# kaiidams/voice100

Measured on AMD Instinct MI355X. Metric: audio frames/sec (fwd+bwd) asr_en_base, B=32x1024-frame mel, higher is better.
Workload: dtype bf16

## Files before the change

### include/voice100_hip.h

```cpp
#ifndef VOICE100_HIP_H
#define VOICE100_HIP_H

#ifdef __cplusplus
extern "C" {
#endif


int v100_dw_num_groups(int B, int C);
int v100_dwconv(const float* x, const float* x2, const float* w, const float* in_a, const float* in_b,
                const float* in_c, int in_mode, float* y, const float* aux, const float* out_a,
                const float* out_b, int out_mode, float* stats, int G, int B, int C, int Tin, int Tout,
                int K, int stride, int pad, int flip, int upsample, int force_generic, void* stream);

int v100_dwconv_wgrad(const float* g, const float* g2, const float* ga, const float* gb, const float* gc,
                      int g_mode, const float* x, const float* xa, const float* xb, int x_mode,
                      float* partial, float* dw, int G, int B, int C, int Tin, int Tout, int K, int stride,
                      int pad, int force_generic, void* stream);

int v100_dwconv_bwd(const float* g, const float* g2, const float* w, const float* ga, const float* gb,
                    const float* gc, const float* xpre, const float* xa, const float* xb, float* dxin,
                    float* stats, float* wpartial, float* dw, int G, int B, int C, int Tin, int Tout, int K,
                    int stride, int pad, int force_split, void* stream);

int v100_pw_num_parts(int B, int T);
int v100_pw_gemm(const float* A, const void* A_bf16, const float* X, const float* X2, const float* xa,
                 const float* xb, const float* xc, int x_mode, float* Y, const float* bias, const float* ea,
                 const float* eb, const float* R, int epi_mode, float* stats, int B, int M, int K, int T,
                 int use_bf16, void* stream);
int v100_pw_gemm_dropmask_supported(int B, int M, int K, int T, int use_bf16);
int v100_pw_gemm_dropmask(const float* A, const void* A_bf16, const float* X, float* Y, const void* keep, float p, int B, int M, int K,
                          int T, int use_bf16, void* stream);

int v100_pw_wgrad_splits(int B, int M, int K);
int v100_pw_wgrad(const float* G, const float* G2, const float* ga, const float* gb, const float* gc, int g_mode,
                  const float* X, const float* xa, const float* xb, int x_mode, float* partial, float* dW,
                  int S, int B, int M, int K, int T, int use_bf16, void* stream);

int v100_weight_prep(const float* w, int rows, int cols, void* w_bf16, float* wt, void* wt_bf16, void* stream);
int v100_weight_prep_f16(const float* w, int rows, int cols, void* w16, void* stream);

int v100_bn_finalize_train(const float* stats, int parts, long long count, const float* gamma, const float* beta,
                           float* running_mean, float* running_var, long long* num_batches_tracked, float momentum,
                           float eps, float* scale, float* shift, float* save_mean, float* save_rstd, int C, void* stream);
int v100_bn_eval_coeffs(const float* gamma, const float* beta, const float* running_mean, const float* running_var,
                        float eps, float* scale, float* shift, int C, void* stream);
int v100_bn_bwd_finalize(const float* partial, int parts, long long count, const float* gamma, const float* mean,
                         const float* rstd, float* p, float* q, float* r, float* dgamma, float* dbeta, int C, void* stream);
int v100_bn_frozen_coeffs(const float* gamma, const float* beta, const float* running_mean, const float* running_var,
                          float eps, float* scale, float* shift, float* mean, float* rstd, int C, void* stream);
int v100_bn_bwd_finalize_frozen(const float* partial, int parts, long long count, const float* gamma, const float* mean,
                                const float* rstd, float* p, float* q, float* r, float* dgamma, float* dbeta, int C, void* stream);

int v100_chan_reduce2(const float* u, const float* v, float* partial, int G, int B, int C, int T, void* stream);
int v100_slab_sum0(const float* partial, int parts, float* out, int C, void* stream);
int v100_chan_affine2(const float* u, const float* v, const float* A, const float* Bc, const float* Cc, float* out,
                      int B, int C, int T, void* stream);
int v100_mul_scale(const float* u, const float* m, float s, float* out, long long n, void* stream);
int v100_dropout_fwd(const float* x, long long seed, float p, float* y, void* mask, long long n, void* stream);
int v100_dropout_bwd(const float* dy, const void* mask, float p, float* dx, long long n, void* stream);
int v100_transpose_last2(const float* in, float* out, int B, int R, int Cc, void* stream);
int v100_embedding_bct(const long long* idx, const float* table, float* out, int B, int V, int C, int T, void* stream);
int v100_embedding_bwd(const long long* idx, const float* g, float* dtable, int B, int V, int C, int T, void* stream);


int v100_augment_fused(const float* x, const int* len, const float* uniform, float* y, int B, int Tin, int Tout,
                       int F, int stretch_rate, float pitch_rate, float amp, int n_tmask, const int* tm_s,
                       const int* tm_e, const float* tm_a, int fm_on, int fm_s, int fm_e, float fm_a, int noise_on,
                       float noise_low, float noise_high, float noise_std, int mix, float log_offset, void* stream);
int v100_augment_fused_len(const float* x, const int* len_raw, int* len_out, int* half_out, const float* uniform, float* y,
                           int B, int Tin, int Tout, int F, int stretch_rate, float pitch_rate, float amp, int n_tmask,
                           const int* tm_s, const int* tm_e, const float* tm_a, int fm_on, int fm_s, int fm_e, float fm_a,
                           int noise_on, float noise_low, float noise_high, float noise_std, int mix, float log_offset,
                           void* stream);
int v100_augment_fused_len_t(const float* x, const int* len_raw, int* len_out, int* half_out, const float* uniform, float* y,
                             float* yt, int B, int Tin, int Tout, int F, int stretch_rate, float pitch_rate, float amp, int n_tmask,
                             const int* tm_s, const int* tm_e, const float* tm_a, int fm_on, int fm_s, int fm_e, float fm_a,
                             int noise_on, float noise_low, float noise_high, float noise_std, int mix, float log_offset,
                             void* stream);

int v100_shift_copy(const float* in, float* out, const float* bias, int B, int C, int Tin, int Tout, int in_ctot,
                    int in_coff, int out_ctot, int out_coff, int in_mul, int in_add, int out_mul, int out_add, int n,
                    int accumulate, void* stream);
int v100_stft_frames(const float* x, float* frames, int B, int N, int T, int hop, int win, int n_fft, void* stream);
int v100_power_spectrum(const float* spec, float* pw, int B, int F, int T, void* stream);
int v100_log_transpose(const float* in, float* out, int B, int C, int T, float offset, void* stream);
int v100_log_mel_fused(const float* x, float* out, const float* window, const float* tw256, const float* tw512, const int* mel_start,
                       const int* mel_count, const float* mel_w, int B, int N, int T, int hop, int n_fft, int n_mels, float log_offset,
                       void* stream);
int v100_log_mel_fused_len(const float* x, const int* lengths, float* out, int* out_len, const float* window, const float* tw256,
                           const float* tw512, const int* mel_start, const int* mel_count, const float* mel_w, int B, int N, int T,
                           int hop, int n_fft, int n_mels, float log_offset, float fill, void* stream);
int v100_world_unnormalize(const float* x, float* f0, float* logspc, float* codeap, const float* f0_mean, const float* f0_std,
                           const float* ls_mean, const float* ls_std, const float* ca_mean, const float* ca_std,
                           int B, int T, int S, int Cap, void* stream);
int v100_world_loss_parts(int B, int Tp);
int v100_world_loss(const float* pred, const float* f0, const float* hasf0, const float* logspc, const float* codeap,
                    const int* length, const float* f0_mean, const float* f0_std, const float* ls_mean, const float* ls_std,
                    const float* ca_mean, const float* ca_std, const float* w, float* partial, float* loss, float* unit,
                    int B, int Tp, int Tt, int S, int Cap, int l1, void* stream);
int v100_world_loss_bwd(const float* unit, const float* gout, float* dpred, int B, int Tp, int S, int Cap, void* stream);
int v100_exp_clip(const float* x, float* y, float offset, long long n, void* stream);

int v100_bct_to_cm(const float* in, float* out, int B, int C, int T, void* stream);
int v100_cm_to_btc(const float* in, float* out, int B, int C, int T, void* stream);

int v100_world_randn_host(float* host_out, long long n);
int v100_world_decode_aperiodicity(const float* coded, float* ap, long long rows, int nb, int fs, int fft_size, void* stream);
long long v100_world_synth_workspace_bytes(int B, int T, int fs, double frame_period_ms, int fft_size, int max_pulses);
int v100_world_synthesize(const float* f0, const float* sp, const float* ap, const float* coded_ap, int nb, const int* frames, const float* randn_table,
                          long long table_len, const float* tw256, const float* tw512, const float* dc_remover, float* y,
                          int* n_pulses, void* workspace, int B, int T, int fs, double frame_period_ms, int fft_size,
                          int max_pulses, void* stream);

int v100_im2col(const float* x, float* cols, int B, int Cin, int Tin, int Tout, int k, int stride, int pad, void* stream);
int v100_col2im(const float* dcols, float* dx, int B, int Cin, int Tin, int Tout, int k, int stride, int pad, void* stream);
int v100_pad_copy(const float* src, float* dst, int B, int C, int Tsrc, int src_step, int src_off, int n, int Tx, int lpad, void* stream);
int v100_pw_taps_supported(int B, int M, int cx, int ntap, int T, int Tx, int use_bf16);
int v100_pw_gemm_taps(const float* A, const void* A_bf16, const float* Xp, float* Y, const float* bias, const float* R,
                      int B, int M, int cx, int T, int Tx, int ntap, const int* shifts, int use_bf16, void* stream);
int v100_pw_wgrad_taps(const float* G, int Tg, int g_off, const float* Xp, float* partial, float* dW, int S, int B, int M,
                       int cx, int T, int Tx, int ntap, const int* shifts, int use_bf16, void* stream);
int v100_ln_num_parts(int B, int T);
int v100_slab_sum2(const float* partial, int parts, float* out0, float* out1, int C, void* stream);
int v100_ln_gelu_fwd(const float* y, const float* gamma, const float* beta, float eps, float* out, float* mean,
                     float* rstd, int B, int C, int T, void* stream);
int v100_ln_gelu_bwd(const float* dout, const float* y, const float* gamma, const float* beta, const float* mean,
                     const float* rstd, float* dy, float* partial, int B, int C, int T, void* stream);

long long v100_launch_count(void);
int v100_copy_probe(const void* src, void* dst, long long nbytes, void* stream);
int v100_timing_enable(int tag_mask);
int v100_timing_read(int tag, double* ms, long long* count, double* bytes);
int v100_rows_copy_probe(const void* src, void* dst, int B, int C, int row_bytes, void* stream);

int v100_pw_gemm_io(const void* A_bf16, const void* X, const void* X2, const float* xa, const float* xb, const float* xc,
                    int x_mode, void* Y, const float* ea, const float* eb, const void* R, int epi_mode, float* stats,
                    int B, int M, int K, int T, int io16, void* stream);
int v100_pw_wgrad_io(const void* G, const void* G2, const float* ga, const float* gb, const float* gc, int g_mode,
                     const void* X, const float* xa, const float* xb, int x_mode, float* partial, float* dW, int S, int B,
                     int M, int K, int T, int io16, void* stream);
int v100_pw_wgrad_group_supported(int B, int M, int K, int T, int S, int g_mode, int x_mode, int io16);
int v100_pw_wgrad_group_tiles(int M, int K, int x_mode);
int v100_pw_wgrad_group(int n, const void* const* ptrs, const int* dims, void* stream);
int v100_pw_wgrad_group_small_supported(int B, int M, int K, int T, int S, int g_mode, int x_mode, int io16);
int v100_pw_wgrad_group_small_tiles(int M, int K, int x_mode);
int v100_pw_wgrad_group_small(int n, const void* const* ptrs, const int* dims, void* stream);
int v100_dw_mfma_supported(int K, int stride);
int v100_row_pitch16(int T, int B);
int v100_dwconv_fwd_train_io(const void* a1, const float* w, const float* in_a, const float* in_b, void* a2, float* stats,
                             int G, int B, int C, int T, int K, int io16, void* stream);
int v100_dwconv_bwd_io(const void* g, const void* g2, const float* w, const float* ga, const float* gb, const float* gc,
                       const void* xpre, const float* xa, const float* xb, void* dxin, float* stats, float* wpartial,
                       float* dw, int G, int B, int C, int T, int K, int io16, void* stream);
int v100_dwconv_bwd_da1_io(const void* g, const void* g2, const float* w, const float* ga, const float* gb, const float* gc,
                           const void* xpre, const float* xa, const float* xb, void* da1_out, float* stats, float* dw,
                           const float* bn1_gamma, const float* bn1_mean, const float* bn1_rstd, float* pqr, float* dgamma,
                           float* dbeta, int B, int C, int T, int K, void* stream);
int v100_dwconv_fwd_eval_io(const void* h1, const float* w, const float* out_a, const float* out_b, void* h2, int B, int C, int T,
                            int K, int flags, void* stream);
int v100_chan_reduce2_io(const void* u, const void* v, float* partial, int G, int B, int C, int T, int io16, void* stream);
int v100_chan_affine2_shadow(const void* u, const float* v, const float* A, const float* Cc, float* out, void* shadow,
                             int B, int C, int T, int u_bf16, void* stream);
int v100_chan_affine2_io(const void* u, const void* v, const float* A, const float* Bc, const float* Cc, void* out,
                         int B, int C, int T, int io16, void* stream);
int v100_ir_act16_supported(const int* shape);

int v100_adam_chunk_elems(void);
int v100_adam_step(const void* chunks, int nchunks, const void* params, const void* grads, const void* exp_avg,
                   const void* exp_avg_sq, double lr, double beta1, double beta2, double eps, double weight_decay, int step,
                   void* stream);

int v100_grad_norm_partials(const void* chunks, int nchunks, const void* grads, void* partials, int norm_type, void* stream);
int v100_adam_step_clip(const void* chunks, int nchunks, const void* params, const void* grads, const void* exp_avg,
                        const void* exp_avg_sq, double lr, double beta1, double beta2, double eps, double weight_decay, int step,
                        int clip_mode, double clip, const void* partials, int npartials, int norm_type, void* total_norm, void* stream);
int v100_grad_clip(const void* chunks, int nchunks, const void* grads, int clip_mode, double clip, const void* partials, int npartials,
                   int norm_type, void* total_norm, void* stream);

int v100_ctc_workspace_floats(int B, int T, int Lmax);
int v100_ctc_loss_mean(const float* logits, const long long* targets, const int* in_len, const int* tgt_len, float* workspace,
                       float* nll, float* loss, float* grad, int B, int T, int V, int Lmax, int blank, void* stream);
int v100_ctc_loss(const float* logits, const long long* targets, const int* in_len, const int* tgt_len, float* workspace,
                  float* nll, float* grad, int B, int T, int V, int Lmax, int blank, void* stream);
int v100_ctc_loss_mean_t(const float* logits, const long long* targets, const int* in_len, const int* tgt_len, float* workspace,
                         float* nll, float* loss, float* grad, int grad_bvt, int B, int T, int V, int Lmax, int blank, void* stream);

enum {
    V100_IR_PREPPED = 1,
    V100_IR_SHADOW_SLOTS = 2,
    V100_IR_FROZEN = 8
};
long long v100_ir_prep_bytes(const int* shape);
long long v100_ir_fwd_workspace_bytes(const int* shape);
long long v100_ir_eval_cache_bytes(const int* shape);
int v100_ir_eval_prep(const int* shape, const void* const* ptrs, void* stream);
int v100_ir_fwd_eval(const int* shape, const void* const* ptrs, void* stream);
int v100_ir_stack_fwd_eval(int n, const int* shapes, const void* const* ptrs, void* stream);
int v100_ir_prep_batched(const int* shapes, const void* const* w1s, const void* const* w3s, void* const* preps, int n, void* stream);
int v100_ir_fwd_train(const int* shape, const void* const* ptrs, void* stream);
long long v100_ir_bwd_workspace_bytes(const int* shape);
int v100_ir_bwd(const int* shape, const void* const* ptrs, void* stream);

long long v100_ir_stack_plan(const int* desc, long long* plan);
int v100_ir_stack_fwd_train(const int* desc, const void* const* params, const void* x, const void* x16, void* blob, void* stream);
int v100_ir_stack_bwd(const int* desc, const void* const* params, const void* x, const void* x16, const void* blob, const void* dy,
                      void* dx, void* grads, void* ws, void* stream);
int v100_ir_stack_wgrad_plan(const int* desc, int have_x16, int min_problem_tiles, int min_flush_tiles, long long* out);
int v100_ir_stack_wgrad_group_thresholds(int min_problem_tiles, int min_flush_tiles);
int v100_ir_stack_wgrad_plan2(const int* desc, int have_x16, int min_problem_tiles, int min_flush_tiles, int min_flush_small, long long* out);
int v100_ir_stack_wgrad_group2_threshold(int min_flush_small);

int v100_ctc_greedy_decode(const float* logits, const int* lens, long long* out, int* out_len, int B, int T, int V, int blank, void* stream);
int v100_ctc_best_path(const float* logp, const long long* labels, const int* in_len, const int* lab_len, void* back_ws, int* path,
                       float* score, int B, int T, int V, int Lmax, int max_move, void* stream);
long long v100_ctc_align_workspace_bytes(int B, int T, int Lmax);
int v100_ctc_align_block(void);
int v100_ctc_align(const float* logp, const long long* labels, const int* in_len, const int* lab_len, void* moves_ws, int* path,
                   long long* best_labels, int* align, float* score, int B, int T, int V, int Lmax, int max_move, void* stream);
long long v100_ctc_align_long_workspace_bytes(int B, int T, int Lmax, int band);
int v100_ctc_align_long_block(void);
int v100_ctc_align_long(const float* logp, const long long* labels, const int* in_len, const int* lab_len, const float* free_logp, void* ws,
                        double* score, int* ok, int* path, int* align, int B, int T, int V, int Lmax, int band, int blank, void* stream);
long long v100_ctc_cut_points_workspace_bytes(int B, int T);
int v100_ctc_cut_points_span(void);
int v100_ctc_cut_points_pass(void);
int v100_ctc_cut_points(const float* logits, const int* lengths, void* ws, int* n_seg, int B, int T, int V, int blank, int max_frames,
                        int min_gap, float margin, int pad, int min_frames, void* stream);
int v100_ctc_cut_points_table(const void* ws, int* start, int* end, int* forced, int B, int T, int S, int pad, void* stream);
long long v100_edit_distance_workspace_bytes(int B, int Th, int Tr);
int v100_edit_distance(const long long* hyp, const int* hyp_len, const long long* ref, const int* ref_len, void* ws, int* dist,
                       int* hyp_n, int* ref_n, long long* totals, int B, int Th, int Tr, int levels, long long sep, void* stream);
long long v100_ctc_beam_workspace_bytes(int B, int T, int V, int W);
int v100_ctc_beam_search(const float* logits, const int* lens, void* ws, long long* ids, int* ids_len, float* scores, int B, int T, int V,
                         int W, int nbest, int blank, void* stream);
int v100_ctc_beam_search_lm(const float* logits, const int* lens, void* ws, long long* ids, int* ids_len, float* scores,
                            const float* lm_logp, const int* lm_next, const float* lm_final, int S, int start_state, float alpha,
                            float beta, int use_eos, float* ctc_scores, float* lm_scores, int B, int T, int V, int W, int nbest,
                            int blank, void* stream);
long long v100_ctc_beam_stream_workspace_bytes(int B, int max_frames, int V, int W);
long long v100_ctc_beam_stream_state_bytes(int B, int W);
int v100_ctc_beam_stream_push(const float* logits, const int* lens, void* ws, void* state, int B, int T, int max_frames, int V, int W,
                              int blank, void* stream);
int v100_ctc_beam_stream_push_lm(const float* logits, const int* lens, void* ws, void* state, const float* lm_logp, const int* lm_next,
                                 const float* lm_final, int S, int start_state, float alpha, float beta, int B, int T, int max_frames,
                                 int V, int W, int blank, void* stream);
int v100_ctc_beam_stream_read(const void* ws, const void* state, long long* ids, int* ids_len, float* scores, int B, int max_frames,
                              int V, int W, int nbest, int width, void* stream);
int v100_ctc_beam_stream_read_lm(const void* ws, const void* state, long long* ids, int* ids_len, float* scores, const float* lm_final,
                                 int S, int start_state, float alpha, float beta, int final, float* ctc_scores, float* lm_scores, int B,
                                 int max_frames, int V, int W, int nbest, int width, void* stream);
long long v100_ctc_segment_workspace_bytes(int B, int T, int Lmax);
int v100_ctc_segment_block(void);
int v100_ctc_segment(const float* logits, const int* in_len, const long long* labels, const int* lab_len, void* ws, float* log_prob,
                     int* start, int* end, float* duration, float* log_conf, int* word_first, int* word_count, int* word_start,
                     int* word_end, float* word_log_conf, int* n_words, int B, int T, int V, int Lmax, int blank, long long sep,
                     void* stream);
long long v100_dtw_workspace_bytes(int B, int Tx, int Ty, int D, int want_path);
int v100_dtw_score(const float* x, const int* x_len, const float* y, const int* y_len, const float* f0x, const float* f0y, void* ws,
                   double* cost, int* path_len, int* voiced, int* vuv_errors, double* f0_sq_cents, double* f0_sq_hz, int* path,
                   double* totals, int B, int Tx, int Ty, int D, int skip, float f0_floor, int mode, void* stream);
int v100_align_expand(const long long* text, const double* align, const int* text_len, long long* out, int* out_len, int B, int Lmax,
                      int Tmax, int head, int tail, void* stream);


int v100_world_randn_host_f64(double* host_out, long long n);
long long v100_world_randn_bound(int kind, int T, int fs, int fft_size);
int v100_world_frames(int fs, int length, double frame_period_ms);
int v100_world_dio_bands(int fs, double f0_floor, double f0_ceil, double channels_in_octave, int* half_lengths, int max_bands);
long long v100_world_dio_workspace_bytes(int B, int max_len, int fs, double f0_floor, double f0_ceil, double channels_in_octave,
                                         double frame_period_ms);
int v100_world_dio(const float* x, const int* lengths, int B, int max_len, int pitch, int fs, double f0_floor, double f0_ceil,
                   double channels_in_octave, double frame_period_ms, double allowed_range, const double* lowcut,
                   const double* nuttall, double* f0, void* workspace, void* stream);
int v100_world_cheaptrick(const float* x, const int* lengths, const double* f0, int B, int max_len, int pitch, int fs,
                          double frame_period_ms, double q1, int fft_size, const double* randn_table, long long table_len,
                          const double* twiddle, double* sp, float* logsp, double log_offset, long long* offsets, void* stream);
long long v100_world_d4c_workspace_bytes(int B, int max_len, int fs, double frame_period_ms);
int v100_world_d4c(const float* x, const int* lengths, const double* f0, int B, int max_len, int pitch, int fs, double frame_period_ms,
                   double threshold, int fft_size, const double* randn_table, long long table_len, const double* twiddle,
                   const double* nuttall, int window_length, double* ap, double* coded, float* coded32, void* workspace, void* stream);

long long v100_lstm_weight_bytes(int H, int ndir, int use_bf16, int backward);
int v100_lstm_geometry(int H, int use_bf16, int backward, int* out);
long long v100_lstm_ws_bytes(int B, int H, int ndir, int backward);
int v100_lstm_sync_words(int B, int ndir);
int v100_lstm_persistent_ok(int B, int H, int ndir, int use_bf16, int backward);
int v100_lstm_weight_prep(const float* w_hh0, const float* w_hh1, int H, int ndir, int use_bf16, int backward, void* out,
                          void* stream);
int v100_lstm_fwd(const float* xproj, const void* w_prep, const float* b_hh0, const float* b_hh1, const int* lens, float* y,
                  float* h_n, float* c_n, float* act, float* cs, float* hprev, void* ws, unsigned* sync, int B, int T, int H,
                  int ndir, int use_bf16, int persistent, void* stream);
int v100_lstm_bwd(const float* dy, const float* dh_n, const float* dc_n, const void* w_prep, const int* lens, const float* act,
                  const float* cs, float* dgates, void* ws, unsigned* sync, int B, int T, int H, int ndir, int use_bf16,
                  int persistent, void* stream);

int v100_world_loss_v2(const float* pred, const float* f0, const float* logspc, const float* codeap, const int* length,
                       const float* f0_mean, const float* f0_std, const float* ls_mean, const float* ls_std,
                       const float* ca_mean, const float* ca_std, float* partial, float* loss, float* unit,
                       int B, int Tp, int Tt, int S, int Cap, int l1, void* stream);
int v100_world_loss_v2_bwd(const float* unit, const float* gout, float* dpred, int B, int Tp, int S, int Cap, void* stream);
int v100_align_loss_parts(int B, int L);
int v100_align_loss(const float* pred, const long long* align, const int* text_len, float* partial, float* loss, float* unit,
                    int B, int L, int W, void* stream);
int v100_align_loss_bwd(const float* unit, const float* gout, float* dpred, int B, int L, void* stream);
int v100_align_expand_v2(const long long* text, const double* align, const int* text_len, long long* out, int* out_len, int B,
                         int Lmax, int Tmax, int head, int tail, void* stream);
int v100_world_unnormalize_v2(const float* x, float* f0, float* logspc, float* codeap, const float* f0_mean, const float* f0_std,
                              const float* ls_mean, const float* ls_std, const float* ca_mean, const float* ca_std,
                              int B, int T, int S, int Cap, void* stream);

int v100_masked_ce_parts(int B, int L);
int v100_masked_ce(const float* logits, const long long* target, const int* target_len, float* partial, float* loss, float* unit,
                   int B, int V, int L, void* stream);
int v100_masked_ce_bwd(const float* unit, const float* gout, float* dlogits, int B, int V, int L, void* stream);

long long v100_resample_out_len(long long len, int o, int n);
int v100_resample_tile(void);
int v100_resample_sinc(const float* x, const int* lens, const float* taps, const int* starts, float* y, int* out_lens, int B,
                       int Nmax, int Mmax, int o, int n, int width, int L, void* stream);

long long v100_flac_workspace_bytes(int B, int S, int H, long long stage_ints);
int v100_flac_decode(const unsigned char* bytes, long long nbytes, const int* table, void* ws, float* wave, int* pcm, int* lengths,
                     int* status, int B, int S, int H, long long stage_ints, int max_file_bytes, int Cw, int Cp, int Nmax, void* stream);

long long v100_flac_encode_workspace_bytes(int F, int C);
int v100_flac_encode(const float* wave, const int* pcm, const int* ftab, void* ws, unsigned char* out, int* report, int* status,
                     int B, int F, int R, int C, long long N, int bits_per_sample, int block_size, int max_lpc_order,
                     int max_partition_order, int rate_code, int rate_extra, long long out_bytes, void* stream);

int v100_world_stat_parts(int B, int T, int S);
int v100_world_stat_accum(const float* f0, const int* f0_len, const float* logspc, const float* codeap, double* partial,
                          double* moments, int B, int T, int S, int A, void* stream);

#ifdef __cplusplus
}
#endif
#endif
```

### voice100_amd/csrc/ctc.hip

```cpp
#include "common.h"
#include <math.h>
#include <type_traits>

#define CTC_CHUNK 64
#define CTC_MAXV 128
#define NEG_INF (-INFINITY)

__device__ __forceinline__ float lse2(float a, float b) {
    const float m = fmaxf(a, b);
    if (m == NEG_INF) return NEG_INF;
    return m + __logf(__expf(a - m) + __expf(b - m));
}
__device__ __forceinline__ float lse3(float a, float b, float c) {
    const float m = fmaxf(fmaxf(a, b), c);
    if (m == NEG_INF) return NEG_INF;
    return m + __logf(__expf(a - m) + __expf(b - m) + __expf(c - m));
}

__global__ void ctc_lse_kernel(const float* __restrict__ logits, float* __restrict__ lse, long rows, int V, int* __restrict__ stall, int B) {
    const long r = (long)blockIdx.x * blockDim.x + threadIdx.x;
    if (r < B) stall[r] = 0;
    if (r >= rows) return;
    const float* p = logits + r * V;
    float m = NEG_INF;
    for (int c = 0; c < V; ++c) m = fmaxf(m, p[c]);
    float s = 0.f;
    for (int c = 0; c < V; ++c) s += expf(p[c] - m);
    lse[r] = m + logf(s);
}

template <int NS>
__global__ __launch_bounds__(256) void ctc_lattice_kernel(const float* __restrict__ logits, const float* __restrict__ lse,
                                                          const long long* __restrict__ targets, const int* __restrict__ in_len,
                                                          const int* __restrict__ tgt_len, float* __restrict__ alpha,
                                                          float* __restrict__ beta, float* __restrict__ nll, int T, int V, int Lmax,
                                                          int Smax, int blank) {
    extern __shared__ float sm[];
    float* lp = sm;
    float* row = sm + CTC_CHUNK * V;
    const int b = blockIdx.x, dir = blockIdx.y, tid = threadIdx.x;
    int Tb = in_len[b];
    if (Tb > T) Tb = T;
    int L = tgt_len[b];
    if (L > Lmax) L = Lmax;
    const int S = 2 * L + 1;
    float* lat = (dir == 0 ? alpha : beta) + (size_t)b * T * Smax;
    const long long* tg = targets + (size_t)b * Lmax;
    const int rs = Smax + 4;
    for (int i = tid; i < 2 * rs; i += 256) row[i] = NEG_INF;
    __syncthreads();
    if (Tb <= 0) { if (dir == 0 && tid == 0) nll[b] = L <= 0 ? 0.f : INFINITY; return; }

    int cls[NS]; bool skip[NS];
#pragma unroll
    for (int k = 0; k < NS; ++k) {
        const int s = tid + 256 * k;
        cls[k] = blank; skip[k] = false;
        if (s < S && (s & 1)) {
            cls[k] = (int)tg[s >> 1];
            if (dir == 0) skip[k] = s >= 2 && tg[s >> 1] != tg[(s >> 1) - 1];
            else skip[k] = s + 2 < S && tg[s >> 1] != tg[(s >> 1) + 1];
        }
        if (cls[k] < 0 || cls[k] >= V) cls[k] = blank;
    }

    const int nchunks = (Tb + CTC_CHUNK - 1) / CTC_CHUNK;
    for (int ci = 0; ci < nchunks; ++ci) {
        const int c0 = dir == 0 ? ci * CTC_CHUNK : (nchunks - 1 - ci) * CTC_CHUNK;
        const int cn = min(CTC_CHUNK, Tb - c0);
        __syncthreads();
        for (int i = tid; i < cn * V; i += 256) {
            const int tt = i / V, c = i - tt * V;
            lp[i] = logits[((size_t)b * T + c0 + tt) * V + c] - lse[(size_t)b * T + c0 + tt];
        }
        __syncthreads();
        for (int j = 0; j < cn; ++j) {
            const int tl = dir == 0 ? j : cn - 1 - j;
            const int t = c0 + tl;
            const bool first = dir == 0 ? (t == 0) : (t == Tb - 1);
            const int cur = t & 1, prv = cur ^ 1;
#pragma unroll
            for (int k = 0; k < NS; ++k) {
                const int s = tid + 256 * k;
                if (s < S) {
                    const float e = lp[tl * V + cls[k]];
                    float v;
                    if (first) {
                        const bool start = dir == 0 ? (s <= 1) : (s >= S - 2);
                        v = start ? e : NEG_INF;
                    } else if (dir == 0) {
                        const float* pr = row + prv * rs + 2 + s;
                        v = e + lse3(pr[0], pr[-1], skip[k] ? pr[-2] : NEG_INF);
                    } else {
                        const float* pr = row + prv * rs + 2 + s;
                        v = e + lse3(pr[0], pr[1], skip[k] ? pr[2] : NEG_INF);
                    }
                    row[cur * rs + 2 + s] = v;
                    lat[(size_t)t * Smax + s] = v;
                }
            }
            __syncthreads();
        }
    }
    if (dir == 0 && tid == 0) {
        const float* last = row + ((Tb - 1) & 1) * rs + 2;
        const float ll = S >= 2 ? lse2(last[S - 1], last[S - 2]) : last[S - 1];
        nll[b] = -ll;
    }
}

__device__ __forceinline__ float ctc_lse3_log2(float a, float b, float c) {
    const float mm = fmaxf(fmaxf(fmaxf(a, b), c), -1e30f);
    const float sum = __builtin_amdgcn_exp2f(a - mm) + __builtin_amdgcn_exp2f(b - mm) + __builtin_amdgcn_exp2f(c - mm);
    return mm + __builtin_amdgcn_logf(sum);
}
#define CTC_RING 32
#define CTC_SPIN_MAX (1 << 20)
#define CTC_PF 8
__device__ __forceinline__ float ctc_wave_shr1(float fill, float v) {
    return __builtin_bit_cast(float, __builtin_amdgcn_update_dpp(__builtin_bit_cast(int, fill), __builtin_bit_cast(int, v), 0x138, 0xf, 0xf, false));
}

__global__ __launch_bounds__(1024) void ctc_lattice_skew_kernel(const float* __restrict__ logits, const float* __restrict__ lse,
                                                                const long long* __restrict__ targets, const int* __restrict__ in_len,
                                                                const int* __restrict__ tgt_len, float* __restrict__ alpha,
                                                                float* __restrict__ beta, float* __restrict__ nll, int T, int V, int Lmax,
                                                                int Smax, int blank, int* __restrict__ stall) {
    __shared__ float bnd[16][CTC_RING][2];
    __shared__ int progress[16];
    __shared__ float fin[2];
    const int b = blockIdx.x, dir = blockIdx.y, tid = threadIdx.x;
    const int w = __builtin_amdgcn_readfirstlane(tid >> 6), lane = tid & 63, NW = blockDim.x >> 6;
    int Tb = in_len[b];
    if (Tb > T) Tb = T;
    int L = tgt_len[b];
    if (L > Lmax) L = Lmax;
    const int S = 2 * L + 1;
    float* lat = (dir == 0 ? alpha : beta) + (size_t)b * T * Smax;
    const long long* tg = targets + (size_t)b * Lmax;
    if (lane == 0) progress[w] = -1;
    if (tid < 2) fin[tid] = NEG_INF;
    __syncthreads();
    if (Tb <= 0) { if (dir == 0 && tid == 0) nll[b] = L <= 0 ? 0.f : INFINITY; return; }

    const int u = tid;
    const int sidx = dir == 0 ? u : S - 1 - u;
    const bool active = u < S;
    int cls = blank;
    bool skip = false;
    if (active && (sidx & 1)) {
        cls = (int)tg[sidx >> 1];
        if (dir == 0) skip = sidx >= 2 && tg[sidx >> 1] != tg[(sidx >> 1) - 1];
        else skip = sidx + 2 < S && tg[sidx >> 1] != tg[(sidx >> 1) + 1];
    }
    if (cls < 0 || cls >= V) cls = blank;

    const float* lg = logits + (size_t)b * T * V + cls;
    const float* ls = lse + (size_t)b * T;
    auto emission = [&](int q) -> float {
        const int qq = q < Tb ? q : Tb - 1;
        const int t = dir == 0 ? qq : Tb - 1 - qq;
        return (lg[(size_t)t * V] - ls[t]) * 1.44269504088896340736f;
    };
    float cur[CTC_PF], nxt[CTC_PF];
#pragma unroll
    for (int j = 0; j < CTC_PF; ++j) cur[j] = emission(j);

    auto prog_load = [&](int i) { return __hip_atomic_load(&progress[i], __ATOMIC_RELAXED, __HIP_MEMORY_SCOPE_WORKGROUP); };
    float a_prev = NEG_INF;
    int pnext = -2;
    float n63 = NEG_INF, n62 = NEG_INF;
    float* lrow = lat + (size_t)(dir == 0 ? 0 : Tb - 1) * Smax + sidx;
    const long lstep = dir == 0 ? (long)Smax : -(long)Smax;
    auto frame = [&](auto up_t, auto down_t, auto first_t, int q, float e) {
        constexpr bool UP = decltype(up_t)::value, DOWN = decltype(down_t)::value, FIRST = decltype(first_t)::value;
        float v63 = NEG_INF, v62 = NEG_INF;
        if constexpr (UP) {
            if constexpr (!FIRST) {
                asm volatile("" : "+v"(pnext));
                if (__builtin_amdgcn_readfirstlane(pnext) >= q - 1) {
                    v63 = n63; v62 = n62;
                } else {
                    const int need = min(q + 1, Tb - 1);
                    int guard = 0;
                    for (; prog_load(w - 1) < need && guard < CTC_SPIN_MAX; ++guard) __builtin_amdgcn_s_sleep(1);
                    if (guard >= CTC_SPIN_MAX && lane == 0) stall[b] = 1;
                    asm volatile("" ::: "memory");
                    v63 = bnd[w - 1][(q - 1) & (CTC_RING - 1)][0];
                    v62 = bnd[w - 1][(q - 1) & (CTC_RING - 1)][1];
                }
            }
            pnext = prog_load(w - 1);
            asm volatile("" ::: "memory");
            n63 = bnd[w - 1][q & (CTC_RING - 1)][0];
            n62 = bnd[w - 1][q & (CTC_RING - 1)][1];
        }
        float v;
        if constexpr (FIRST) {
            v = (u <= 1) ? e : NEG_INF;
        } else {
            const float sm1 = ctc_wave_shr1(v63, a_prev);
            const float sm2 = ctc_wave_shr1(v62, sm1);
            v = e + ctc_lse3_log2(a_prev, sm1, skip ? sm2 : NEG_INF);
        }
        if (!active) v = NEG_INF;
        if constexpr (DOWN) {
            if ((q & (CTC_RING / 2 - 1)) == 0 && q >= CTC_RING / 2) {
                int guard = 0;
                for (; prog_load(w + 1) < q - CTC_RING / 2 && guard < CTC_SPIN_MAX; ++guard) __builtin_amdgcn_s_sleep(1);
                if (guard >= CTC_SPIN_MAX && lane == 0) stall[b] = 1;
            }
            asm volatile("" ::: "memory");
            if (lane >= 62) bnd[w][q & (CTC_RING - 1)][63 - lane] = v;
        }
        asm volatile("" ::: "memory");
        if (lane == 0) __hip_atomic_store(&progress[w], q, __ATOMIC_RELAXED, __HIP_MEMORY_SCOPE_WORKGROUP);
        a_prev = v;
        if (active) *lrow = v * 0.69314718055994530942f;
        lrow += lstep;
    };
    auto run = [&](auto up_t, auto down_t) {
        for (int q0 = 0; q0 < Tb; q0 += CTC_PF) {
#pragma unroll
            for (int j = 0; j < CTC_PF; ++j) nxt[j] = emission(q0 + CTC_PF + j);
            if (q0 == 0) {
                frame(up_t, down_t, std::true_type{}, 0, cur[0]);
#pragma unroll
                for (int j = 1; j < CTC_PF; ++j)
                    if (j < Tb) frame(up_t, down_t, std::false_type{}, j, cur[j]);
            } else if (q0 + CTC_PF <= Tb) {
#pragma unroll
                for (int j = 0; j < CTC_PF; ++j) frame(up_t, down_t, std::false_type{}, q0 + j, cur[j]);
            } else {
#pragma unroll
                for (int j = 0; j < CTC_PF; ++j)
                    if (q0 + j < Tb) frame(up_t, down_t, std::false_type{}, q0 + j, cur[j]);
            }
#pragma unroll
            for (int j = 0; j < CTC_PF; ++j) cur[j] = nxt[j];
        }
    };
    const bool has_up = w > 0, has_down = w < NW - 1;
    if (has_up && has_down) run(std::true_type{}, std::true_type{});
    else if (has_up) run(std::true_type{}, std::false_type{});
    else if (has_down) run(std::false_type{}, std::true_type{});
    else run(std::false_type{}, std::false_type{});
    if (dir == 0) {
        if (u == S - 1) fin[0] = a_prev;
        if (S >= 2 && u == S - 2) fin[1] = a_prev;
        __syncthreads();
        if (tid == 0) nll[b] = -(S >= 2 ? lse2(fin[0] * 0.69314718055994530942f, fin[1] * 0.69314718055994530942f) : fin[0] * 0.69314718055994530942f);
    }
}

template <int NW, bool BVT>
__global__ __launch_bounds__(64 * NW) void ctc_grad_kernel(const float* __restrict__ logits, const float* __restrict__ lse,
                                                           const long long* __restrict__ targets, const int* __restrict__ in_len,
                                                           const int* __restrict__ tgt_len, const float* __restrict__ alpha,
                                                           const float* __restrict__ beta, float* nll,
                                                           float* __restrict__ grad, int B, int T, int V, int Lmax, int Smax, int blank,
                                                           int mean_scale, const int* __restrict__ stall, float* __restrict__ loss) {
    __shared__ float bins[2 * NW][CTC_MAXV];
    __shared__ float stage[BVT ? NW : 1][BVT ? CTC_MAXV : 1];
    const int wave = threadIdx.x >> 6, lane = threadIdx.x & 63;
    const long w = (long)blockIdx.x * NW + wave;
    if (loss && blockIdx.x == 0 && wave == 0) {
        float s = 0.f;
        for (int bb = lane; bb < B; bb += 64) {
            const float v = stall[bb] ? __builtin_nanf("") : nll[bb];
            if (!(v == INFINITY || v == -INFINITY)) s += v / (float)max(tgt_len[bb], 1);
        }
        s = wave_sum(s);
        if (lane == 0) loss[0] = s / (float)B;
    }
    const auto frame = [&]() {
    const int b = (int)(w / T), t = (int)(w % T);
    float* g = BVT ? &stage[wave][0] : grad + ((size_t)b * T + t) * V;
    if (stall[b]) {
        for (int c = lane; c < V; c += 64) g[c] = __builtin_nanf("");
        if (t == 0 && lane == 0) nll[b] = __builtin_nanf("");
        return;
    }
    const float n = nll[b];
    int Tb = in_len[b];
    if (Tb > T) Tb = T;
    if (t >= Tb || !(n < INFINITY)) {
        for (int c = lane; c < V; c += 64) g[c] = 0.f;
        return;
    }
    int L = tgt_len[b];
    if (L > Lmax) L = Lmax;
    const int S = 2 * L + 1;
    const float* al = alpha + ((size_t)b * T + t) * Smax;
    const float* be = beta + ((size_t)b * T + t) * Smax;
    const long long* tg = targets + (size_t)b * Lmax;
    unsigned* dmin = reinterpret_cast<unsigned*>(&bins[NW + wave][0]);
    for (int c = lane; c < V; c += 64) { bins[wave][c] = 0.f; dmin[c] = 0x7f800000u; }
    float m = NEG_INF;
    for (int s = lane; s < S; s += 64) m = fmaxf(m, al[s] + be[s]);
#pragma unroll
    for (int off = 32; off > 0; off >>= 1) m = fmaxf(m, __shfl_xor(m, off, 64));
    __builtin_amdgcn_wave_barrier();
    asm volatile("" ::: "memory");
    if (m > NEG_INF) {
        for (int s = lane; s < S; s += 64) {
            int c = (s & 1) ? (int)tg[s >> 1] : blank;
            if (c < 0 || c >= V) c = blank;
            const float d = m - (al[s] + be[s]);
            if (d >= 0.f) atomicMin(&dmin[c], __builtin_bit_cast(unsigned, d));
        }
        __builtin_amdgcn_wave_barrier();
        asm volatile("" ::: "memory");
        for (int s = lane; s < S; s += 64) {
            int c = (s & 1) ? (int)tg[s >> 1] : blank;
            if (c < 0 || c >= V) c = blank;
            const float dm = __builtin_bit_cast(float, dmin[c]);
            const float x = al[s] + be[s];
            if (dm < INFINITY || x != x) atomicAdd(&bins[wave][c], expf((x - m) + dm));
        }
    }
    __builtin_amdgcn_wave_barrier();
    asm volatile("" ::: "memory");
    const float z = lse[(size_t)b * T + t];
    const float* lg = logits + ((size_t)b * T + t) * V;
    const float gs = mean_scale ? 1.f / ((float)max(tgt_len[b], 1) * (float)B) : 1.f;
    for (int c = lane; c < V; c += 64) {
        const float lpc = lg[c] - z;
        const float acc = bins[wave][c];
        const float dm = __builtin_bit_cast(float, dmin[c]);
        const float occ = (acc > 0.f) ? expf(((m - dm) + n - lpc) + logf(acc)) : (acc != acc ? acc : 0.f);
        g[c] = (expf(lpc) - occ) * gs;
    }
    };
    if (w < (long)B * T) frame();
    if constexpr (BVT) {
        __syncthreads();
        const long w0 = (long)blockIdx.x * NW;
        for (int i = threadIdx.x; i < V * NW; i += 64 * NW) {
            const int c = i / NW, j = i % NW;
            const long wj = w0 + j;
            if (wj < (long)B * T) grad[((size_t)(wj / T) * V + c) * T + (wj % T)] = stage[j][c];
        }
    }
}

extern "C" int v100_ctc_workspace_floats(int B, int T, int Lmax) {
    const long n = 2L * B * T * (2 * Lmax + 1) + (long)B * T + B;
    return n > 0x7fffffffL ? -1 : (int)n;
}

static int ctc_run(const float* logits, const long long* targets, const int* in_len, const int* tgt_len, float* workspace, float* nll,
                   float* loss, float* grad, int grad_bvt, int B, int T, int V, int Lmax, int blank, void* stream);

extern "C" int v100_ctc_loss(const float* logits, const long long* targets, const int* in_len, const int* tgt_len, float* workspace,
                             float* nll, float* grad, int B, int T, int V, int Lmax, int blank, void* stream) {
    return ctc_run(logits, targets, in_len, tgt_len, workspace, nll, nullptr, grad, 0, B, T, V, Lmax, blank, stream);
}

extern "C" int v100_ctc_loss_mean(const float* logits, const long long* targets, const int* in_len, const int* tgt_len, float* workspace,
                                  float* nll, float* loss, float* grad, int B, int T, int V, int Lmax, int blank, void* stream) {
    if (!loss) return V100_ERR_NULL;
    return ctc_run(logits, targets, in_len, tgt_len, workspace, nll, loss, grad, 0, B, T, V, Lmax, blank, stream);
}

extern "C" int v100_ctc_loss_mean_t(const float* logits, const long long* targets, const int* in_len, const int* tgt_len,
                                    float* workspace, float* nll, float* loss, float* grad, int grad_bvt, int B, int T, int V, int Lmax,
                                    int blank, void* stream) {
    if (!loss) return V100_ERR_NULL;
    return ctc_run(logits, targets, in_len, tgt_len, workspace, nll, loss, grad, grad_bvt ? 1 : 0, B, T, V, Lmax, blank, stream);
}

static int ctc_run(const float* logits, const long long* targets, const int* in_len, const int* tgt_len, float* workspace, float* nll,
                   float* loss, float* grad, int grad_bvt, int B, int T, int V, int Lmax, int blank, void* stream) {
    if (!logits || !targets || !in_len || !tgt_len || !workspace || !nll || !grad) return V100_ERR_NULL;
    if (B <= 0 || T <= 0 || V <= 0 || V > CTC_MAXV || Lmax < 0 || 2 * Lmax + 1 > 4096 || blank < 0 || blank >= V) return V100_ERR_SHAPE;
    hipStream_t st = (hipStream_t)stream;
    const int Smax = 2 * Lmax + 1;
    float* alpha = workspace;
    float* beta = alpha + (size_t)B * T * Smax;
    float* lse = beta + (size_t)B * T * Smax;
    const long rows = (long)B * T;
    int* stall = (int*)(lse + (size_t)B * T);
    const size_t shmem = (size_t)(CTC_CHUNK * V + 2 * (Smax + 4)) * sizeof(float);
    if (Smax > 2048 && shmem > 65536 &&
        hipFuncSetAttribute((const void*)ctc_lattice_kernel<16>, hipFuncAttributeMaxDynamicSharedMemorySize, (int)shmem) != hipSuccess) {
        (void)hipGetLastError();
        return V100_ERR_LAUNCH;
    }
    V100_GGL(ctc_lse_kernel, dim3((unsigned)((rows + 255) / 256)), dim3(256), 0, st, logits, lse, rows, V, stall, B);
#define CTC_LATTICE(NS_)                                                                                                          \
    V100_GGL(ctc_lattice_kernel<NS_>, dim3(B, 2), dim3(256), shmem, st, logits, lse, targets, in_len, tgt_len, alpha, beta, \
                       nll, T, V, Lmax, Smax, blank)
    if (Smax <= 1024) {
        const int nw = (Smax + 63) / 64;
        V100_GGL(ctc_lattice_skew_kernel, dim3(B, 2), dim3(64 * nw), 0, st, logits, lse, targets, in_len, tgt_len, alpha, beta,
                           nll, T, V, Lmax, Smax, blank, stall);
    } else if (Smax <= 2048) { CTC_LATTICE(8); }
    else { CTC_LATTICE(16); }
#undef CTC_LATTICE
    if (grad_bvt) V100_GGL((ctc_grad_kernel<16, true>), dim3((unsigned)((rows + 15) / 16)), dim3(1024), 0, st, logits, lse, targets, in_len, tgt_len,
                           alpha, beta, nll, grad, B, T, V, Lmax, Smax, blank, loss ? 1 : 0, stall, loss);
    else V100_GGL((ctc_grad_kernel<4, false>), dim3((unsigned)((rows + 3) / 4)), dim3(256), 0, st, logits, lse, targets, in_len, tgt_len,
                  alpha, beta, nll, grad, B, T, V, Lmax, Smax, blank, loss ? 1 : 0, stall, loss);
    return v100_launch_status();
}
```

Before: 10.72 million.

## Batch CTC lattice inter-wave boundary exchange into groups of frames

Adds a grouped variant of the skewed CTC alpha/beta lattice kernel. Each wave computes G frames (default 16) before publishing its lane-63 boundary values to the next wave as float4 vectors, so progress flags and spin-waits happen once per group instead of once per frame. It also drops the second boundary value (lane 62) because the skip term only needs one shifted neighbour. Per-wave skew latency grows to a group of frames, and the grouped path is selected by a heuristic based on T and the wave count, with an override setter.

```diff
diff --git a/include/voice100_hip.h b/include/voice100_hip.h
--- a/include/voice100_hip.h
+++ b/include/voice100_hip.h
@@ -184,6 +184,9 @@
                   float* nll, float* grad, int B, int T, int V, int Lmax, int blank, void* stream);
 int v100_ctc_loss_mean_t(const float* logits, const long long* targets, const int* in_len, const int* tgt_len, float* workspace,
                          float* nll, float* loss, float* grad, int grad_bvt, int B, int T, int V, int Lmax, int blank, void* stream);
+int v100_ctc_lattice_plan(int T, int Lmax);
+int v100_ctc_lattice_ring_frames(void);
+int v100_ctc_lattice_form(int form);
 
 enum {
     V100_IR_PREPPED = 1,
diff --git a/voice100_amd/csrc/ctc.hip b/voice100_amd/csrc/ctc.hip
--- a/voice100_amd/csrc/ctc.hip
+++ b/voice100_amd/csrc/ctc.hip
@@ -117,16 +117,24 @@
 #define CTC_RING 32
 #define CTC_SPIN_MAX (1 << 20)
 #define CTC_PF 8
+#ifndef CTC_GROUP
+#define CTC_GROUP 16
+#endif
+#define CTC_GRING 8
+static_assert(CTC_GROUP % 4 == 0 && CTC_GROUP >= 4 && CTC_GROUP <= 16, "the group's edge values travel as float4");
+typedef float ctc_f4 __attribute__((ext_vector_type(4)));
 __device__ __forceinline__ float ctc_wave_shr1(float fill, float v) {
     return __builtin_bit_cast(float, __builtin_amdgcn_update_dpp(__builtin_bit_cast(int, fill), __builtin_bit_cast(int, v), 0x138, 0xf, 0xf, false));
 }
 
+template <int G>
 __global__ __launch_bounds__(1024) void ctc_lattice_skew_kernel(const float* __restrict__ logits, const float* __restrict__ lse,
                                                                 const long long* __restrict__ targets, const int* __restrict__ in_len,
                                                                 const int* __restrict__ tgt_len, float* __restrict__ alpha,
                                                                 float* __restrict__ beta, float* __restrict__ nll, int T, int V, int Lmax,
                                                                 int Smax, int blank, int* __restrict__ stall) {
-    __shared__ float bnd[16][CTC_RING][2];
+    constexpr int PF = G > 0 ? G : CTC_PF;
+    __shared__ __attribute__((aligned(16))) float bnd[16][G > 0 ? CTC_GRING * G : CTC_RING];
     __shared__ int progress[16];
     __shared__ float fin[2];
     const int b = blockIdx.x, dir = blockIdx.y, tid = threadIdx.x;
@@ -162,48 +170,51 @@
         const int t = dir == 0 ? qq : Tb - 1 - qq;
         return (lg[(size_t)t * V] - ls[t]) * 1.44269504088896340736f;
     };
-    float cur[CTC_PF], nxt[CTC_PF];
-#pragma unroll
-    for (int j = 0; j < CTC_PF; ++j) cur[j] = emission(j);
+    auto settle = [](float (&e)[PF]) {
+#pragma unroll
+        for (int j = 0; j < PF; ++j) asm volatile("" : "+v"(e[j]));
+    };
+    float cur[PF], nxt[PF];
+#pragma unroll
+    for (int j = 0; j < PF; ++j) cur[j] = emission(j);
+    settle(cur);
 
     auto prog_load = [&](int i) { return __hip_atomic_load(&progress[i], __ATOMIC_RELAXED, __HIP_MEMORY_SCOPE_WORKGROUP); };
     float a_prev = NEG_INF;
-    int pnext = -2;
-    float n63 = NEG_INF, n62 = NEG_INF;
     float* lrow = lat + (size_t)(dir == 0 ? 0 : Tb - 1) * Smax + sidx;
     const long lstep = dir == 0 ? (long)Smax : -(long)Smax;
+    auto step = [&](float edge, float e) {
+        const float sm1 = ctc_wave_shr1(edge, a_prev);
+        const float sm2 = ctc_wave_shr1(NEG_INF, sm1);
+        const float v = e + ctc_lse3_log2(a_prev, sm1, skip ? sm2 : NEG_INF);
+        return active ? v : NEG_INF;
+    };
+    int pnext = -2;
+    float n63 = NEG_INF;
     auto frame = [&](auto up_t, auto down_t, auto first_t, int q, float e) {
         constexpr bool UP = decltype(up_t)::value, DOWN = decltype(down_t)::value, FIRST = decltype(first_t)::value;
-        float v63 = NEG_INF, v62 = NEG_INF;
+        float v63 = NEG_INF;
         if constexpr (UP) {
             if constexpr (!FIRST) {
                 asm volatile("" : "+v"(pnext));
                 if (__builtin_amdgcn_readfirstlane(pnext) >= q - 1) {
-                    v63 = n63; v62 = n62;
+                    v63 = n63;
                 } else {
                     const int need = min(q + 1, Tb - 1);
                     int guard = 0;
                     for (; prog_load(w - 1) < need && guard < CTC_SPIN_MAX; ++guard) __builtin_amdgcn_s_sleep(1);
                     if (guard >= CTC_SPIN_MAX && lane == 0) stall[b] = 1;
                     asm volatile("" ::: "memory");
-                    v63 = bnd[w - 1][(q - 1) & (CTC_RING - 1)][0];
-                    v62 = bnd[w - 1][(q - 1) & (CTC_RING - 1)][1];
+                    v63 = bnd[w - 1][(q - 1) & (CTC_RING - 1)];
                 }
             }
             pnext = prog_load(w - 1);
             asm volatile("" ::: "memory");
-            n63 = bnd[w - 1][q & (CTC_RING - 1)][0];
-            n62 = bnd[w - 1][q & (CTC_RING - 1)][1];
+            n63 = bnd[w - 1][q & (CTC_RING - 1)];
         }
         float v;
-        if constexpr (FIRST) {
-            v = (u <= 1) ? e : NEG_INF;
-        } else {
-            const float sm1 = ctc_wave_shr1(v63, a_prev);
-            const float sm2 = ctc_wave_shr1(v62, sm1);
-            v = e + ctc_lse3_log2(a_prev, sm1, skip ? sm2 : NEG_INF);
-        }
-        if (!active) v = NEG_INF;
+        if constexpr (FIRST) v = (active && u <= 1) ? e : NEG_INF;
+        else v = step(v63, e);
         if constexpr (DOWN) {
             if ((q & (CTC_RING / 2 - 1)) == 0 && q >= CTC_RING / 2) {
                 int guard = 0;
@@ -211,7 +222,7 @@
                 if (guard >= CTC_SPIN_MAX && lane == 0) stall[b] = 1;
             }
             asm volatile("" ::: "memory");
-            if (lane >= 62) bnd[w][q & (CTC_RING - 1)][63 - lane] = v;
+            if (lane == 63) bnd[w][q & (CTC_RING - 1)] = v;
         }
         asm volatile("" ::: "memory");
         if (lane == 0) __hip_atomic_store(&progress[w], q, __ATOMIC_RELAXED, __HIP_MEMORY_SCOPE_WORKGROUP);
@@ -219,25 +230,89 @@
         if (active) *lrow = v * 0.69314718055994530942f;
         lrow += lstep;
     };
+    auto group = [&](auto up_t, auto down_t, auto full_t, int g, int n) {
+        constexpr bool UP = decltype(up_t)::value, DOWN = decltype(down_t)::value, FULL = decltype(full_t)::value;
+        constexpr int G4 = G / 4;
+        ctc_f4 edge[G4 > 0 ? G4 : 1];
+        for (int i = 0; i < G4; ++i) edge[i] = ctc_f4{NEG_INF, NEG_INF, NEG_INF, NEG_INF};
+        if constexpr (UP) {
+            const ctc_f4* slot = reinterpret_cast<const ctc_f4*>(&bnd[w - 1][(g & (CTC_GRING - 1)) * G]);
+            const int p = prog_load(w - 1);
+            asm volatile("" ::: "memory");
+#pragma unroll
+            for (int i = 0; i < G4; ++i) edge[i] = slot[i];
+#pragma unroll
+            for (int i = 0; i < G4; ++i) asm volatile("" : "+v"(edge[i]));
+            if (__builtin_amdgcn_readfirstlane(p) < g) {
+                int guard = 0;
+                for (; prog_load(w - 1) < g && guard < CTC_SPIN_MAX; ++guard) __builtin_amdgcn_s_sleep(1);
+                if (guard >= CTC_SPIN_MAX && lane == 0) stall[b] = 1;
+                asm volatile("" ::: "memory");
+#pragma unroll
+                for (int i = 0; i < G4; ++i) edge[i] = slot[i];
+            }
+        }
+        const float* ev = reinterpret_cast<const float*>(edge);
+        float val[G > 0 ? G : 1];
+        const float carried = a_prev;
+#pragma unroll
+        for (int j = 0; j < G; ++j) {
+            val[j] = a_prev;
+            if (FULL || j < n) {
+                if (!FULL && g == 0 && j == 0) val[j] = (active && u <= 1) ? cur[0] : NEG_INF;
+                else val[j] = step(ev[j], cur[j]);
+            }
+            asm volatile("" : "+v"(val[j]));
+            a_prev = val[j];
+        }
+        if constexpr (DOWN) {
+            if ((g & (CTC_GRING / 2 - 1)) == 0 && g >= CTC_GRING / 2) {
+                int guard = 0;
+                for (; prog_load(w + 1) < g - CTC_GRING / 2 && guard < CTC_SPIN_MAX; ++guard) __builtin_amdgcn_s_sleep(1);
+                if (guard >= CTC_SPIN_MAX && lane == 0) stall[b] = 1;
+            }
+            asm volatile("" ::: "memory");
+            if (lane == 63) {
+                ctc_f4* slot = reinterpret_cast<ctc_f4*>(&bnd[w][(g & (CTC_GRING - 1)) * G]);
+#pragma unroll
+                for (int i = 0; i < G4; ++i)
+                    slot[i] = ctc_f4{i == 0 ? carried : val[4 * i - 1], val[4 * i], val[4 * i + 1], val[4 * i + 2]};
+            }
+        }
+        if constexpr (UP || DOWN) {
+            asm volatile("" ::: "memory");
+            if (lane == 0) __hip_atomic_store(&progress[w], g, __ATOMIC_RELAXED, __HIP_MEMORY_SCOPE_WORKGROUP);
+        }
+        if (active) {
+#pragma unroll
+            for (int j = 0; j < G; ++j)
+                if (FULL || j < n) lrow[j * lstep] = val[j] * 0.69314718055994530942f;
+        }
+        lrow += G * lstep;
+    };
     auto run = [&](auto up_t, auto down_t) {
-        for (int q0 = 0; q0 < Tb; q0 += CTC_PF) {
-#pragma unroll
-            for (int j = 0; j < CTC_PF; ++j) nxt[j] = emission(q0 + CTC_PF + j);
-            if (q0 == 0) {
+        for (int q0 = 0; q0 < Tb; q0 += PF) {
+#pragma unroll
+            for (int j = 0; j < PF; ++j) nxt[j] = emission(q0 + PF + j);
+            if constexpr (G > 0) {
+                if (q0 > 0 && q0 + G <= Tb) group(up_t, down_t, std::true_type{}, q0 / G, G);
+                else group(up_t, down_t, std::false_type{}, q0 / G, min(G, Tb - q0));
+            } else if (q0 == 0) {
                 frame(up_t, down_t, std::true_type{}, 0, cur[0]);
 #pragma unroll
-                for (int j = 1; j < CTC_PF; ++j)
+                for (int j = 1; j < PF; ++j)
                     if (j < Tb) frame(up_t, down_t, std::false_type{}, j, cur[j]);
-            } else if (q0 + CTC_PF <= Tb) {
-#pragma unroll
-                for (int j = 0; j < CTC_PF; ++j) frame(up_t, down_t, std::false_type{}, q0 + j, cur[j]);
+            } else if (q0 + PF <= Tb) {
+#pragma unroll
+                for (int j = 0; j < PF; ++j) frame(up_t, down_t, std::false_type{}, q0 + j, cur[j]);
             } else {
 #pragma unroll
-                for (int j = 0; j < CTC_PF; ++j)
+                for (int j = 0; j < PF; ++j)
                     if (q0 + j < Tb) frame(up_t, down_t, std::false_type{}, q0 + j, cur[j]);
             }
 #pragma unroll
-            for (int j = 0; j < CTC_PF; ++j) cur[j] = nxt[j];
+            for (int j = 0; j < PF; ++j) cur[j] = nxt[j];
+            settle(cur);
         }
     };
     const bool has_up = w > 0, has_down = w < NW - 1;
@@ -349,6 +424,24 @@
     return n > 0x7fffffffL ? -1 : (int)n;
 }
 
+static int ctc_lattice_form = -1;
+static bool ctc_lattice_rule(int T, int nw) { return T >= 32 + 4 * nw; }
+static bool ctc_lattice_grouped(int T, int nw) { return ctc_lattice_form >= 0 ? ctc_lattice_form != 0 : ctc_lattice_rule(T, nw); }
+
+extern "C" int v100_ctc_lattice_form(int form) {
+    if (form < -1 || form > 1) return V100_ERR_SHAPE;
+    ctc_lattice_form = form;
+    return V100_OK;
+}
+
+extern "C" int v100_ctc_lattice_plan(int T, int Lmax) {
+    const int Smax = 2 * Lmax + 1;
+    if (T <= 0 || Lmax < 0 || Smax > 1024) return -1;
+    return ctc_lattice_rule(T, (Smax + 63) / 64) ? CTC_GROUP : 0;
+}
+
+extern "C" int v100_ctc_lattice_ring_frames(void) { return CTC_GRING * CTC_GROUP; }
+
 static int ctc_run(const float* logits, const long long* targets, const int* in_len, const int* tgt_len, float* workspace, float* nll,
                    float* loss, float* grad, int grad_bvt, int B, int T, int V, int Lmax, int blank, void* stream);
 
@@ -393,8 +486,12 @@
                        nll, T, V, Lmax, Smax, blank)
     if (Smax <= 1024) {
         const int nw = (Smax + 63) / 64;
-        V100_GGL(ctc_lattice_skew_kernel, dim3(B, 2), dim3(64 * nw), 0, st, logits, lse, targets, in_len, tgt_len, alpha, beta,
-                           nll, T, V, Lmax, Smax, blank, stall);
+        if (ctc_lattice_grouped(T, nw))
+            V100_GGL(ctc_lattice_skew_kernel<CTC_GROUP>, dim3(B, 2), dim3(64 * nw), 0, st, logits, lse, targets, in_len, tgt_len, alpha,
+                     beta, nll, T, V, Lmax, Smax, blank, stall);
+        else
+            V100_GGL(ctc_lattice_skew_kernel<0>, dim3(B, 2), dim3(64 * nw), 0, st, logits, lse, targets, in_len, tgt_len, alpha, beta,
+                     nll, T, V, Lmax, Smax, blank, stall);
     } else if (Smax <= 2048) { CTC_LATTICE(8); }
     else { CTC_LATTICE(16); }
 #undef CTC_LATTICE
```

After: 10.88 million (median of 6 runs). 1.01x the previous value.
